# OminiX-ai/OminiX-MLX

Measured on AMD Instinct MI355X. Metric: decode_tokens_per_sec, higher is better.
Workload: dtype bf16

## Files before the change

### ominix-mlx_amd/csrc/attn_step.hip

```cpp
#include <algorithm>

#include "attn.hpp"
#include "act16.hpp"
#include "gemv_parts.hpp"
#include "granule.hpp"
#include "launch_timing.hpp"

namespace omx {

namespace {

constexpr int kBlock = 512;
constexpr int kWaves = 8;

template <int N>
__device__ __forceinline__ float swap_halves(float v) {
    if (N == 16) return dpp_f<0x128>(v);
    return dpp_f<0x1B>(dpp_f<kDppHalfMirror>(v));
}

template <bool F16 = false>
__device__ __forceinline__ void unpack8(const u32x4 r, float (&x)[8]) {
#pragma unroll
    for (int e = 0; e < 4; ++e) {
        x[2 * e] = Act16<F16>::lo(r[e]);
        x[2 * e + 1] = Act16<F16>::hi(r[e]);
    }
}

template <int D, int NB, bool F16 = false>
__device__ __forceinline__ void gather_head(const AttnStepArgs& a, const uint64_t* base, int n_active, unsigned tag, int lane,
                                            int dim, bf16_t* out, uint64_t* xg_head) {
    constexpr int STRIDE = D + 2;
    unsigned long long ml0 = 0, ml1 = 0, og[NB][16];
    bool ok_ml = false, ok_b[NB];
#pragma unroll
    for (int b = 0; b < NB; ++b) ok_b[b] = b * 16 >= n_active;
    const int sl = min(lane, n_active - 1);
    for (unsigned spins = 0;; ++spins) {
        if (!ok_ml) {
            ml0 = ld_granule(base + (size_t)sl * STRIDE + D);
            ml1 = ld_granule(base + (size_t)sl * STRIDE + D + 1);
        }
#pragma unroll
        for (int b = 0; b < NB; ++b) {
            if (ok_b[b]) continue;
#pragma unroll
            for (int j = 0; j < 16; ++j) og[b][j] = ld_granule(base + (size_t)min(b * 16 + j, n_active - 1) * STRIDE + dim);
        }
        bool all = true;
        if (!ok_ml) ok_ml = __all((unsigned)(ml0 >> 32) == tag && (unsigned)(ml1 >> 32) == tag);
        all = ok_ml;
#pragma unroll
        for (int b = 0; b < NB; ++b) {
            if (!ok_b[b]) {
                bool ok = true;
#pragma unroll
                for (int j = 0; j < 16; ++j) ok &= (unsigned)(og[b][j] >> 32) == tag;
                ok_b[b] = __all(ok);
            }
            all = all && ok_b[b];
        }
        if (all) break;
        if (spins >= kGranuleSpinLimit) {
            if (lane == 0) __hip_atomic_store(a.abort_flag, 1u, __ATOMIC_RELAXED, __HIP_MEMORY_SCOPE_AGENT);
            break;
        }
        __builtin_amdgcn_s_sleep(1);
    }
    const float m = lane < n_active ? __uint_as_float((unsigned)ml0) : -INFINITY;
    const float l = lane < n_active ? __uint_as_float((unsigned)ml1) : 0.f;
    const float M = wave_max(m);
    const float f = (m == -INFINITY) ? 0.f : __expf(m - M);
    const float L = wave_sum(f * l);
    float acc = 0.f;
#pragma unroll
    for (int b = 0; b < NB; ++b) {
        if (b * 16 >= n_active) break;
#pragma unroll
        for (int j = 0; j < 16; ++j)
            acc = fmaf(readlane_f(f, b * 16 + j), __uint_as_float((unsigned)og[b][j]), acc);
    }
    const bf16_t r = Act16<F16>::bits(acc / L);
    out[dim] = r;
    if (xg_head) {
        const float nb = dpp_f<kDppXor1>(bf16_to_f32(r));
        if (!(lane & 1)) st_granule_u32(xg_head + dim / 2, tag, (unsigned)r | ((unsigned)f32_to_bf16(nb) << 16));
    }
}

typedef __attribute__((ext_vector_type(2))) __bf16 bf16x2_t;
typedef __attribute__((ext_vector_type(2))) float f32x2;

typedef __attribute__((ext_vector_type(8))) __bf16 bf16x8_t;
__device__ __forceinline__ float dot8_bf16(const u32x4 a, const u32x4 b) {
    const bf16x8_t A = __builtin_bit_cast(bf16x8_t, a), B = __builtin_bit_cast(bf16x8_t, b);
    float d = 0.f;
    d = __builtin_amdgcn_fdot2_f32_bf16(__builtin_shufflevector(A, A, 0, 1), __builtin_shufflevector(B, B, 0, 1), d, false);
    d = __builtin_amdgcn_fdot2_f32_bf16(__builtin_shufflevector(A, A, 2, 3), __builtin_shufflevector(B, B, 2, 3), d, false);
    d = __builtin_amdgcn_fdot2_f32_bf16(__builtin_shufflevector(A, A, 4, 5), __builtin_shufflevector(B, B, 4, 5), d, false);
    d = __builtin_amdgcn_fdot2_f32_bf16(__builtin_shufflevector(A, A, 6, 7), __builtin_shufflevector(B, B, 6, 7), d, false);
    return d;
}

constexpr int kKU = 3;

template <bool F16>
__device__ __forceinline__ float dot8_16(const u32x4 a, const u32x4 b) {
    if constexpr (!F16) return dot8_bf16(a, b);
    float d = 0.f;
#pragma unroll
    for (int e = 0; e < 4; ++e) d = Act16<true>::dot2(a[e], b[e], d);
    return d;
}

constexpr int kORows = 4;

constexpr int kGuBlockPairs = 48, kGuHidden = 4096, kGuNV = kGuHidden / 512;
enum { kGuTicket = 0, kGuReduced = 1, kGuWords = 4 };

__device__ __forceinline__ int gateup_claim(int* sm_gu, int lane) {
    int t = 0;
    if (lane == 0) t = __hip_atomic_fetch_add(sm_gu + kGuTicket, 1, __ATOMIC_RELAXED, __HIP_MEMORY_SCOPE_WORKGROUP);
    return __builtin_amdgcn_readfirstlane(t);
}

__device__ __forceinline__ void gateup_issue(const AttnStepArgs& a, u32x4 (*w)[kGuNV], int pair, int lane) {
    const u32x4* g = reinterpret_cast<const u32x4*>(a.gu_gate + (size_t)pair * kGuHidden);
    const u32x4* u = reinterpret_cast<const u32x4*>(a.gu_up + (size_t)pair * kGuHidden);
#pragma unroll
    for (int j = 0; j < kGuNV; ++j) {
        w[0][j] = ld_nt(g + j * 64 + lane);
        w[1][j] = ld_nt(u + j * 64 + lane);
    }
    __builtin_amdgcn_sched_barrier(0);
}

template <int NVW>
__device__ __forceinline__ void oproj_await_vector(const AttnStepArgs& a, u32x4* sm_x, unsigned tag, int lane, int wave) {
    asm volatile("s_waitcnt vmcnt(0)" ::: "memory");
    if (wave == 0) {
        constexpr int SEGS = NVW * 8;
        const uint64_t* probe = a.xg + (size_t)min(lane, SEGS - 1) * 32 + 31;
        for (unsigned spins = 0; spins < kGranuleSpinLimit; ++spins) {
            const unsigned long long g = ld_granule(probe);
            if (__all((unsigned)(g >> 32) == tag)) break;
            __builtin_amdgcn_s_sleep(4);
        }
    }
    __syncthreads();
    constexpr int GP = (NVW + 1) / 2;
    static_assert((NVW * 256) % GP == 0, "a thread takes all of its granules or none");
    bool done = (int)threadIdx.x * GP >= NVW * 256;
    unsigned* sx = reinterpret_cast<unsigned*>(sm_x);
    for (unsigned spins = 0;; ++spins) {
        if (!done) {
            unsigned long long g[GP];
#pragma unroll
            for (int i = 0; i < GP; ++i) g[i] = ld_granule(a.xg + (size_t)threadIdx.x * GP + i);
            bool ok = true;
#pragma unroll
            for (int i = 0; i < GP; ++i) ok &= (unsigned)(g[i] >> 32) == tag;
            if (ok) {
#pragma unroll
                for (int i = 0; i < GP; ++i) sx[threadIdx.x * GP + i] = (unsigned)g[i];
                done = true;
            }
        }
        if (__syncthreads_and(done)) break;
        if (spins >= kGranuleSpinLimit) {
            if (threadIdx.x == 0) __hip_atomic_store(a.abort_flag, 1u, __ATOMIC_RELAXED, __HIP_MEMORY_SCOPE_AGENT);
            break;
        }
        __builtin_amdgcn_s_sleep(2);
    }
}

template <bool DN = false>
__device__ __forceinline__ void gateup_reduce(const AttnStepArgs& a, const u32x4 (*w)[kGuNV], const u32x4* xs, int pair, int lane,
                                              uint16_t* park = nullptr) {
    typedef Act16<false> A;
    float acc[2];
    rows_dot<false, 2, kGuNV>(w, xs, lane, acc);
    if constexpr (DN) {
        if (lane == 0) {
            const uint16_t v = epi_bits<EPI_SWIGLU, A>(acc[0], acc[1], (bf16_t)0, 0);
            a.gu_out[pair] = v;
            *park = v;
        }
    } else
    if (lane == 0) a.gu_out[pair] = epi_bits<EPI_SWIGLU, A>(acc[0], acc[1], (bf16_t)0, 0);
}

constexpr int kDnInter = 12288, kDnBlockRows = 16, kDnNV = kDnInter / 512 / 4, kDnUnits = kDnBlockRows / 2 * 4, kDnQRows = 3;
constexpr int kDnPartOff = kDnInter * 2, kDnParkOff = kDnPartOff + kDnBlockRows * 4 * 4, kDnLdsBytes = kDnParkOff + kGuBlockPairs * 2;
enum { kDnTicket = 4, kDnReduced = 5, kDnStored = 6, kDnWords = 8 };

__device__ __forceinline__ int down_claim(int* sm_gu, int lane) {
    int t = 0;
    if (lane == 0) t = __hip_atomic_fetch_add(sm_gu + kDnTicket, 1, __ATOMIC_RELAXED, __HIP_MEMORY_SCOPE_WORKGROUP);
    return __builtin_amdgcn_readfirstlane(t);
}

__device__ __forceinline__ void down_issue(const AttnStepArgs& a, u32x4 (*w)[kDnNV], int row_begin, int u, int lane) {
    const u32x4* p = reinterpret_cast<const u32x4*>(a.dn_w) + (size_t)(row_begin + 2 * (u >> 2)) * (kDnInter / 8) + (u & 3) * (kDnNV * 64) + lane;
#pragma unroll
    for (int r = 0; r < 2; ++r) {
#pragma unroll
        for (int j = 0; j < kDnNV; ++j) w[r][j] = ld_nt(p + (size_t)r * (kDnInter / 8) + j * 64);
    }
    __builtin_amdgcn_sched_barrier(0);
}

__device__ __forceinline__ void down_reduce(const u32x4 (*w)[kDnNV], const u32x4* xa, float* part, int u, int lane) {
    float acc[2];
    rows_dot<false, 2, kDnNV>(w, xa + (u & 3) * (kDnNV * 64), lane, acc);
    if (lane == 0) {
#pragma unroll
        for (int r = 0; r < 2; ++r) part[(2 * (u >> 2) + r) * 4 + (u & 3)] = acc[r];
    }
}

template <bool TRACE>
__device__ __forceinline__ void down_qkv_phase(const AttnStepArgs& a, unsigned char* sm_dn, u32x4* xs, float* red, int* sm_gu, unsigned res2,
                                               unsigned tag, int lane, int wave, unsigned long long* tr) {
    typedef Act16<false> A;
    u32x4* xa = reinterpret_cast<u32x4*>(sm_dn);
    float* part = reinterpret_cast<float*>(sm_dn + kDnPartOff);
    const int blk = (int)blockIdx.y * (int)gridDim.x + (int)blockIdx.x;
    const int row_begin = blk * kDnBlockRows;
    const int q_row0 = (blk * kWaves + __builtin_amdgcn_readfirstlane(wave)) * kDnQRows;
    constexpr int PV = kGuNV * 64 / 256;
    u32x4 nwv[PV];
#pragma unroll
    for (int i = 0; i < PV; ++i) nwv[i] = *(reinterpret_cast<const u32x4*>(a.nq_norm_w) + (threadIdx.x & 255) + i * 256);
    bf16_t ob[kDnQRows];
#pragma unroll
    for (int r = 0; r < kDnQRows; ++r) ob[r] = *(a.nq_bias ? a.nq_bias + min(q_row0 + r, a.nq.rows - 1) : a.nq_norm_w);
    u32x4 dA[2][kDnNV], dB[2][kDnNV];
    int tA = 0, tB = 0;
    u32x4 qw[kDnQRows][kGuNV];
    auto issue_qkv = [&](const int r0, const int r1) {
#pragma unroll
        for (int r = r0; r < r1; ++r) {
            const u32x4* p = reinterpret_cast<const u32x4*>(a.nq.row_ptr(min(q_row0 + r, a.nq.rows - 1), kGuHidden));
#pragma unroll
            for (int j = 0; j < kGuNV; ++j) qw[r][j] = ld_nt(p + j * 64 + lane);
        }
        __builtin_amdgcn_sched_barrier(0);
    };
    const bool sweeper = (wave & (kWaves / 2 - 1)) == 0;
    lds_barrier();
    if (wave == 0 && lane < kGuBlockPairs / 2)
        st_granule_u32(a.ag + (size_t)blk * (kGuBlockPairs / 2) + lane, tag, reinterpret_cast<const unsigned*>(sm_dn + kDnParkOff)[lane]);
    lds_barrier();
    if (sweeper) {
        constexpr int HALF = kDnInter / 2 / 2, GPL = HALF / 64;
        const int half = __builtin_amdgcn_readfirstlane(wave) / (kWaves / 2);
        const uint64_t* gr = a.ag + (size_t)half * HALF;
        for (unsigned spins = 0; spins < kGranuleSpinLimit; ++spins) {
            const unsigned long long g = ld_granule(gr + (size_t)lane * GPL + (GPL - 1));
            if (__all((unsigned)(g >> 32) == tag)) break;
            __builtin_amdgcn_s_sleep(4);
        }
        unsigned long long g[GPL];
#pragma unroll
        for (int i = 0; i < GPL; ++i) g[i] = ld_granule(gr + (size_t)i * 64 + lane);
        __builtin_amdgcn_sched_barrier(0);
        lds_barrier();
        tA = down_claim(sm_gu, lane);
        down_issue(a, dA, row_begin, tA, lane);
        unsigned bad = 0;
#pragma unroll
        for (int i = 0; i < GPL; ++i) bad |= (unsigned)(g[i] >> 32) ^ tag;
        asm volatile("; activation vector: tags read behind the first down unit" : "+v"(bad));
        if (!__all(bad == 0)) {
            for (unsigned spins = 0;; ++spins) {
#pragma unroll
                for (int i = 0; i < GPL; ++i) g[i] = ld_granule(gr + (size_t)i * 64 + lane);
                bool ok = true;
#pragma unroll
                for (int i = 0; i < GPL; ++i) ok &= (unsigned)(g[i] >> 32) == tag;
                if (__all(ok)) break;
                if (spins >= kGranuleSpinLimit) {
                    if (lane == 0) __hip_atomic_store(a.abort_flag, 1u, __ATOMIC_RELAXED, __HIP_MEMORY_SCOPE_AGENT);
                    break;
                }
                __builtin_amdgcn_s_sleep(4);
            }
        }
        unsigned* sx = reinterpret_cast<unsigned*>(xa) + half * HALF;
#pragma unroll
        for (int i = 0; i < GPL; ++i) sx[i * 64 + lane] = (unsigned)g[i];
        if (TRACE && threadIdx.x == 0) tr[11] = wall_clock64();
        tB = down_claim(sm_gu, lane);
        down_issue(a, dB, row_begin, tB, lane);
        issue_qkv(0, kDnQRows - 1);
    } else {
        tA = down_claim(sm_gu, lane);
        down_issue(a, dA, row_begin, tA, lane);
        tB = down_claim(sm_gu, lane);
        down_issue(a, dB, row_begin, tB, lane);
        issue_qkv(0, 1);
        lds_barrier();
        issue_qkv(1, kDnQRows - 1);
    }
    lds_barrier();
    down_reduce(dA, xa, part, tA, lane);
    if (TRACE && threadIdx.x == 0) tr[12] = wall_clock64();
    int n_reduced = 1;
    int nA = down_claim(sm_gu, lane), nB;
    for (;;) {
        if (nA >= kDnUnits) {
            down_reduce(dB, xa, part, tB, lane);
            ++n_reduced;
            break;
        }
        tA = nA;
        down_issue(a, dA, row_begin, tA, lane);
        nB = down_claim(sm_gu, lane);
        down_reduce(dB, xa, part, tB, lane);
        if (nB >= kDnUnits) {
            down_reduce(dA, xa, part, tA, lane);
            n_reduced += 2;
            break;
        }
        tB = nB;
        down_issue(a, dB, row_begin, tB, lane);
        nA = down_claim(sm_gu, lane);
        down_reduce(dA, xa, part, tA, lane);
        n_reduced += 2;
    }
    if (TRACE && lane == 0) __hip_atomic_fetch_add(sm_gu + kDnReduced, n_reduced, __ATOMIC_RELAXED, __HIP_MEMORY_SCOPE_WORKGROUP);
    issue_qkv(kDnQRows - 1, kDnQRows);
    lds_barrier();
    if (wave == 0) {
        if (lane < kDnBlockRows / 2) {
            const uint32_t o2 = residual_pair<A, 4>(part + 2 * lane * 4, res2);
            reinterpret_cast<uint32_t*>(a.dn_out)[row_begin / 2 + lane] = o2;
            st_granule_u32(a.rg + row_begin / 2 + lane, tag, o2);
        }
        sweep_granules<kGuHidden / 2, 1>(a.rg, reinterpret_cast<unsigned*>(xs), 0, tag, lane, a.abort_flag);
        if (TRACE && lane == 0) tr[13] = wall_clock64();
    }
    lds_barrier();
    rmsnorm_in_lds<A, PV>(xs, red, nwv, kGuHidden, a.eps, threadIdx.x < 256);
    float acc[kDnQRows];
    rows_dot<false, kDnQRows, kGuNV>(qw, xs, lane, acc);
    if (lane == 0) {
        int stored = 0;
#pragma unroll
        for (int r = 0; r < kDnQRows; ++r)
            if (q_row0 + r < a.nq.rows) {
                a.nq_out[q_row0 + r] = A::bits(a.nq_bias ? acc[r] + A::val(ob[r]) : acc[r]);
                ++stored;
            }
        if (TRACE) __hip_atomic_fetch_add(sm_gu + kDnStored, stored, __ATOMIC_RELAXED, __HIP_MEMORY_SCOPE_WORKGROUP);
    }
    if constexpr (TRACE) {
        lds_barrier();
        if (threadIdx.x == 0) {
            tr[14] = wall_clock64();
            tr[15] = (unsigned long long)sm_gu[kDnReduced] | (unsigned long long)sm_gu[kDnStored] << 32;
        }
    }
}

template <bool TRACE, bool DN = false>
__device__ __forceinline__ void gateup_phase(const AttnStepArgs& a, u32x4* xs, float* red, int* sm_gu, const uint16_t* sm_pub, unsigned tag,
                                             int lane, int wave, int pub_row0, int pub_rows, unsigned long long* tr,
                                             unsigned char* sm_dn = nullptr) {
    typedef Act16<false> A;
    const int pair0 = ((int)blockIdx.y * (int)gridDim.x + (int)blockIdx.x) * kGuBlockPairs;
    uint16_t* park = DN ? reinterpret_cast<uint16_t*>(sm_dn + kDnParkOff) : nullptr;
    constexpr int PV = kGuNV * 64 / 256;
    u32x4 nwv[PV];
#pragma unroll
    for (int i = 0; i < PV; ++i) nwv[i] = *(reinterpret_cast<const u32x4*>(a.gu_norm_w) + (threadIdx.x & 255) + i * 256);
    u32x4 wA[2][kGuNV], wB[2][kGuNV];
    int tA = 0, tB;
    if (wave != 0) {
        tA = gateup_claim(sm_gu, lane);
        gateup_issue(a, wA, pair0 + tA, lane);
    }
    lds_barrier();
    if (wave == 0) {
        if (lane < pub_rows / 2) st_granule_u32(a.hg + pub_row0 / 2 + lane, tag, reinterpret_cast<const unsigned*>(sm_pub)[lane]);
        constexpr int GPL = kGuHidden / 2 / 64;
        for (unsigned spins = 0; spins < kGranuleSpinLimit; ++spins) {
            const unsigned long long g = ld_granule(a.hg + (size_t)lane * GPL + (GPL - 1));
            if (__all((unsigned)(g >> 32) == tag)) break;
            __builtin_amdgcn_s_sleep(4);
        }
        unsigned long long g[GPL];
#pragma unroll
        for (int i = 0; i < GPL; ++i) g[i] = ld_granule(a.hg + (size_t)i * 64 + lane);
        __builtin_amdgcn_sched_barrier(0);
        lds_barrier();
        tA = gateup_claim(sm_gu, lane);
        gateup_issue(a, wA, pair0 + tA, lane);
        unsigned bad = 0;
#pragma unroll
        for (int i = 0; i < GPL; ++i) bad |= (unsigned)(g[i] >> 32) ^ tag;
        asm volatile("; hidden row: tags read behind the first (gate, up) pair" : "+v"(bad));
        if (!__all(bad == 0)) {
            for (unsigned spins = 0;; ++spins) {
#pragma unroll
                for (int i = 0; i < GPL; ++i) g[i] = ld_granule(a.hg + (size_t)i * 64 + lane);
                bool ok = true;
#pragma unroll
                for (int i = 0; i < GPL; ++i) ok &= (unsigned)(g[i] >> 32) == tag;
                if (__all(ok)) break;
                if (spins >= kGranuleSpinLimit) {
                    if (lane == 0) __hip_atomic_store(a.abort_flag, 1u, __ATOMIC_RELAXED, __HIP_MEMORY_SCOPE_AGENT);
                    break;
                }
                __builtin_amdgcn_s_sleep(4);
            }
        }
        unsigned* sx = reinterpret_cast<unsigned*>(xs);
#pragma unroll
        for (int i = 0; i < GPL; ++i) sx[i * 64 + lane] = (unsigned)g[i];
        if (TRACE && lane == 0 && pub_rows > 0) tr[4] = wall_clock64();
        tB = gateup_claim(sm_gu, lane);
    } else {
        lds_barrier();
        tB = gateup_claim(sm_gu, lane);
        gateup_issue(a, wB, pair0 + tB, lane);
    }
    lds_barrier();
    unsigned res2 = 0;
    if constexpr (DN) res2 = reinterpret_cast<const unsigned*>(xs)[(pair0 / kGuBlockPairs) * (kDnBlockRows / 2) + (lane & (kDnBlockRows / 2 - 1))];
    rmsnorm_in_lds<A, PV>(xs, red, nwv, kGuHidden, a.eps, threadIdx.x < 256);
    if (wave == 0) {
        gateup_issue(a, wB, pair0 + tB, lane);
        gateup_reduce<DN>(a, wA, xs, pair0 + tA, lane, park + tA);
        if (TRACE && threadIdx.x == 0) tr[7] = wall_clock64();
        asm volatile("; first pair reduced: wave 0, its second pair just asked for" ::: "memory");
    } else {
        gateup_reduce<DN>(a, wA, xs, pair0 + tA, lane, park + tA);
        asm volatile("; first pair reduced: the second pair came in through the hop" ::: "memory");
    }
    int n_reduced = 1;
    int nA = gateup_claim(sm_gu, lane), nB;
    for (;;) {
        if (nA >= kGuBlockPairs) {
            gateup_reduce<DN>(a, wB, xs, pair0 + tB, lane, park + tB);
            ++n_reduced;
            break;
        }
        tA = nA;
        gateup_issue(a, wA, pair0 + tA, lane);
        nB = gateup_claim(sm_gu, lane);
        gateup_reduce<DN>(a, wB, xs, pair0 + tB, lane, park + tB);
        if (nB >= kGuBlockPairs) {
            gateup_reduce<DN>(a, wA, xs, pair0 + tA, lane, park + tA);
            n_reduced += 2;
            break;
        }
        tB = nB;
        gateup_issue(a, wB, pair0 + tB, lane);
        nA = gateup_claim(sm_gu, lane);
        gateup_reduce<DN>(a, wA, xs, pair0 + tA, lane, park + tA);
        n_reduced += 2;
    }
    if constexpr (TRACE) {
        if (lane == 0) {
            __hip_atomic_fetch_add(sm_gu + kGuReduced, n_reduced, __ATOMIC_RELAXED, __HIP_MEMORY_SCOPE_WORKGROUP);
            if (wave == 0) tr[8] = wall_clock64();
            if (wave == kWaves - 1) tr[9] = wall_clock64();
        }
        lds_barrier();
        if (threadIdx.x == 0) tr[10] = (unsigned long long)sm_gu[kGuReduced];
    }
    if constexpr (DN) down_qkv_phase<TRACE>(a, sm_dn, xs, red, sm_gu, res2, tag, lane, wave, tr);
}

template <int NVW, int R, bool GU = false>
__device__ __forceinline__ void oproj_phase(const AttnStepArgs& a, u32x4* sm_x, unsigned tag, int lane, int wave, int o_row0,
                                            unsigned long long* tr, uint16_t* sm_pub = nullptr, int pub_row0 = 0) {
    u32x4 ow[R][NVW];
#pragma unroll
    for (int r = 0; r < R; ++r) {
        const int row = min(o_row0 + r, a.o_rows - 1);
        const u32x4* p = reinterpret_cast<const u32x4*>(a.o_w + (size_t)row * (NVW * 512));
#pragma unroll
        for (int j = 0; j < NVW; ++j) ow[r][j] = __builtin_nontemporal_load(p + j * 64 + lane);
    }
    bf16_t o_res[R];
#pragma unroll
    for (int r = 0; r < R; ++r) o_res[r] = a.o_resid[min(o_row0 + r, a.o_rows - 1)];
    __builtin_amdgcn_sched_barrier(0);
    oproj_await_vector<NVW>(a, sm_x, tag, lane, wave);
    if (tr && threadIdx.x == 0) tr[5] = wall_clock64();
    float acc[R];
    rows_dot<false, R, NVW>(ow, sm_x, lane, acc);
    if (lane == 0) {
#pragma unroll
        for (int r = 0; r < R; ++r)
            if (o_row0 + r < a.o_rows) {
                if (a.o_out_f32) a.o_out_f32[o_row0 + r] = acc[r];
                else {
                    const bf16_t hb = f32_to_bf16(bf16_to_f32(o_res[r]) + round_bf16(acc[r]));
                    a.o_out[o_row0 + r] = hb;
                    if (GU) sm_pub[o_row0 + r - pub_row0] = hb;
                }
            }
    }
    if (tr && threadIdx.x == 0) tr[6] = wall_clock64();
}


template <int NVW, int R>
__device__ __forceinline__ void oproj_phase_q4(const AttnStepArgs& a, u32x4* sm_x, float* sm_xsum, unsigned tag, int lane, int wave,
                                               int o_row0, unsigned long long* tr) {
    static_assert(NVW % 4 == 0, "K must be a multiple of 2048");
    constexpr int ST = NVW / 4;
    u32x4 ow[R][ST];
    uint32_t sbv[R][ST];
    const int words_per_row = NVW * 64, groups_per_row = NVW * 512 / a.o_group;
#pragma unroll
    for (int r = 0; r < R; ++r) {
        const int row = min(o_row0 + r, a.o_rows - 1);
        const uint32_t* p = a.o_wq + (size_t)row * words_per_row;
        const uint32_t* psb = a.o_sb + (size_t)row * groups_per_row;
#pragma unroll
        for (int st = 0; st < ST; ++st) {
            const int chunk = st * 64 + lane;
            ow[r][st] = __builtin_nontemporal_load(reinterpret_cast<const u32x4*>(p + (size_t)chunk * 4));
            sbv[r][st] = psb[chunk * 32 / a.o_group];
        }
    }
    bf16_t o_res[R];
#pragma unroll
    for (int r = 0; r < R; ++r) o_res[r] = a.o_resid[min(o_row0 + r, a.o_rows - 1)];
    __builtin_amdgcn_sched_barrier(0);
    oproj_await_vector<NVW>(a, sm_x, tag, lane, wave);
    if ((int)threadIdx.x < NVW * 64) {
        const u32x4 o = sm_x[threadIdx.x];
        u32x4 t;
        t[0] = __builtin_amdgcn_perm(o[1], o[0], 0x05040100u); t[1] = __builtin_amdgcn_perm(o[3], o[2], 0x05040100u);
        t[2] = __builtin_amdgcn_perm(o[1], o[0], 0x07060302u); t[3] = __builtin_amdgcn_perm(o[3], o[2], 0x07060302u);
        sm_x[threadIdx.x] = t;
        float sv = 0.f;
#pragma unroll
        for (int q = 0; q < 4; ++q) sv += bf16lo(o[q]) + bf16hi(o[q]);
        sv += dpp_f<kDppXor1>(sv);
        sv += dpp_f<kDppXor2>(sv);
        if ((threadIdx.x & 3) == 0) sm_xsum[threadIdx.x >> 2] = sv;
    }
    __syncthreads();
    if (tr && threadIdx.x == 0) tr[5] = wall_clock64();
    float acc[R];
#pragma unroll
    for (int r = 0; r < R; ++r) acc[r] = 0.f;
#pragma unroll
    for (int st = 0; st < ST; ++st) {
        const int chunk = st * 64 + lane;
        uint32_t xp[16];
#pragma unroll
        for (int j = 0; j < 4; ++j) {
            const u32x4 xv = sm_x[chunk * 4 + j];
#pragma unroll
            for (int q = 0; q < 4; ++q) xp[j * 4 + q] = xv[q];
        }
        const float xsm = sm_xsum[chunk];
#pragma unroll
        for (int r = 0; r < R; ++r) {
            float d = 0.f;
            const float scl = bf16lo(sbv[r][st]);
            float bia = bf16hi(sbv[r][st]);
#pragma unroll
            for (int wi = 0; wi < 4; ++wi) {
                const uint32_t wdw = ow[r][st][wi];
                const uint32_t lo = wdw & 0x0F0F0F0Fu, hi = (wdw >> 4) & 0x0F0F0F0Fu;
                const uint32_t c43 = 0x43434343u;
                const uint32_t q0 = __builtin_amdgcn_perm(c43, lo, 0x04010400u), q1 = __builtin_amdgcn_perm(c43, lo, 0x04030402u);
                const uint32_t q2 = __builtin_amdgcn_perm(c43, hi, 0x04010400u), q3 = __builtin_amdgcn_perm(c43, hi, 0x04030402u);
                d = __builtin_amdgcn_fdot2_f32_bf16(__builtin_bit_cast(bf16x2_t, xp[wi * 4 + 0]), __builtin_bit_cast(bf16x2_t, q0), d, false);
                d = __builtin_amdgcn_fdot2_f32_bf16(__builtin_bit_cast(bf16x2_t, xp[wi * 4 + 1]), __builtin_bit_cast(bf16x2_t, q1), d, false);
                d = __builtin_amdgcn_fdot2_f32_bf16(__builtin_bit_cast(bf16x2_t, xp[wi * 4 + 2]), __builtin_bit_cast(bf16x2_t, q2), d, false);
                d = __builtin_amdgcn_fdot2_f32_bf16(__builtin_bit_cast(bf16x2_t, xp[wi * 4 + 3]), __builtin_bit_cast(bf16x2_t, q3), d, false);
            }
            bia = fmaf(-128.0f, scl, bia);
            acc[r] = fmaf(scl, d, acc[r]);
            acc[r] = fmaf(bia, xsm, acc[r]);
        }
    }
#pragma unroll
    for (int r = 0; r < R; ++r) acc[r] = wave_sum(acc[r]);
    if (lane == 0) {
#pragma unroll
        for (int r = 0; r < R; ++r)
            if (o_row0 + r < a.o_rows) a.o_out[o_row0 + r] = f32_to_bf16(bf16_to_f32(o_res[r]) + round_bf16(acc[r]));
    }
    if (tr && threadIdx.x == 0) tr[6] = wall_clock64();
}


template <int D, int GT, bool TRACE, int NVW, bool F16 = false, bool GU = false, bool DN = false>
__global__ __launch_bounds__(kBlock, 1) void attn_step_kernel(const AttnStepArgs a) {
    static_assert(!DN || GU, "down + the next q/k/v follow gate/up only");
    static_assert(!F16 || NVW == 0, "the O projection rides in the launch for bfloat16 models only");
    static_assert(!GU || (NVW == kGuNV && D == 128), "gate/up follows the bf16 O projection of hidden 4096 only");
    typedef Act16<F16> A16;
    constexpr int LPR = D / 8;
    constexpr int TPW = 64 / LPR;
    constexpr bool QO = NVW >= 100;
    constexpr int NV = QO ? NVW - 100 : NVW;
    constexpr bool OPROJ = NV > 0;
    extern __shared__ __attribute__((aligned(16))) unsigned char smem[];
    float* sm_o = reinterpret_cast<float*>(smem);
    float* sm_m = sm_o + kWaves * TPW * GT * D;
    float* sm_l = sm_m + kWaves * GT;
    u32x4* sm_q = reinterpret_cast<u32x4*>(sm_l + kWaves * GT);
    u32x4* sm_x = sm_q + (GT + 1) * LPR;
    float* sm_xsum = reinterpret_cast<float*>(sm_x + NV * 64);
    int* sm_gu = reinterpret_cast<int*>(sm_x + NV * 64);

    const int lane = threadIdx.x & 63;
    const int wave = threadIdx.x >> 6;
    const int c = lane % LPR;
    const int sg = lane / LPR;
    const int kvh = blockIdx.x, split = blockIdx.y;
    const int G = a.H / a.Hkv;
    unsigned long long* tr = TRACE ? a.trace + ((size_t)split * a.Hkv + kvh) * kAttnTraceWords : nullptr;
    if (TRACE && threadIdx.x == 0) tr[0] = wall_clock64();
    if constexpr (GU) {
        if (threadIdx.x < (DN ? kDnWords : kGuWords)) sm_gu[threadIdx.x] = 0;
    }

    bf16_t* Kb = a.k + (size_t)kvh * a.kv_head_stride;
    bf16_t* Vb = a.v + (size_t)kvh * a.kv_head_stride;
    const int t_begin = split * a.chunk;
    const int n_units = a.chunk / TPW;

    const bf16_t* kraw = a.qkv + (size_t)a.H * D + (size_t)kvh * D;
    const bool does_q = wave < GT, does_k = wave == GT % kWaves;
    const bf16_t* my_raw = does_q ? a.qkv + (size_t)(kvh * G + min(wave, G - 1)) * D : kraw;
    const u32x4 raw0 = *reinterpret_cast<const u32x4*>(my_raw + c * 8);
    const u32x4 raw1 = *reinterpret_cast<const u32x4*>(kraw + c * 8);
    const u32x4 vnew = *reinterpret_cast<const u32x4*>(kraw + (size_t)a.Hkv * D + c * 8);
    const int i0 = (c % (LPR / 2)) * 8;
    const f32x4* cp = reinterpret_cast<const f32x4*>(a.rope_cur + i0);
    const f32x4* sp = reinterpret_cast<const f32x4*>(a.rope_cur + D / 2 + i0);
    const f32x4 c0 = cp[0], c1 = cp[1], s0 = sp[0], s1 = sp[1];
    u32x4 wq_raw = {0, 0, 0, 0}, wk_raw = {0, 0, 0, 0};
    if (a.q_norm_w) {
        wq_raw = *reinterpret_cast<const u32x4*>(a.q_norm_w + c * 8);
        wk_raw = *reinterpret_cast<const u32x4*>(a.k_norm_w + c * 8);
    }
    u32x4 kr[kKU], vr[kKU];
    auto issue_kv = [&](int u0) {
#pragma unroll
        for (int u = 0; u < kKU; ++u) {
            const int tc = min(t_begin + (u0 + u * kWaves) * TPW + sg, a.cap - 1);
            kr[u] = *reinterpret_cast<const u32x4*>(Kb + (size_t)tc * D + c * 8);
            vr[u] = *reinterpret_cast<const u32x4*>(Vb + (size_t)tc * D + c * 8);
        }
    };
    issue_kv(wave);
    const int pos = *a.pos_ptr;
    const unsigned tag = *a.seq_ptr * a.tag_mul + a.tag_add;

    {
        float cs[8], sn[8];
#pragma unroll
        for (int e = 0; e < 4; ++e) {
            cs[e] = c0[e]; cs[4 + e] = c1[e];
            sn[e] = s0[e]; sn[4 + e] = s1[e];
        }
        const bool first_half = c < LPR / 2;
        auto norm_rope = [&](const u32x4 raw, const u32x4 w_raw) -> u32x4 {
            float x[8], w[8];
            unpack8<F16>(raw, x);
            unpack8<F16>(w_raw, w);
            float ss = 0.f;
#pragma unroll
            for (int e = 0; e < 8; ++e) ss = fmaf(x[e], x[e], ss);
            ss = group_sum<LPR>(ss);
            const float rstd = a.q_norm_w ? 1.0f / sqrtf(ss / (float)D + a.eps) : 1.0f;
            float y[8];
#pragma unroll
            for (int e = 0; e < 8; ++e) {
                const float xn = a.q_norm_w ? A16::rnd(x[e] * rstd * w[e]) : x[e];
                const float other = swap_halves<LPR>(xn);
                y[e] = first_half ? xn * cs[e] - other * sn[e] : other * sn[e] + xn * cs[e];
            }
            u32x4 out;
#pragma unroll
            for (int e = 0; e < 4; ++e) out[e] = A16::pack(y[2 * e], y[2 * e + 1]);
            return out;
        };
        if (does_q && sg == 0) sm_q[wave * LPR + c] = norm_rope(raw0, wq_raw);
        if (does_k && sg == 0) sm_q[GT * LPR + c] = norm_rope(does_q ? raw1 : raw0, wk_raw);
    }
    asm volatile("s_waitcnt lgkmcnt(0)\n\ts_barrier" ::: "memory");
    u32x4 q[GT];
#pragma unroll
    for (int g = 0; g < GT; ++g) q[g] = sm_q[g * LPR + c];
    const u32x4 knew = sm_q[GT * LPR + c];

    const int Tk = pos + 1;
    const int n_active = (Tk + a.chunk - 1) / a.chunk;
    const int t_end = min(Tk, t_begin + a.chunk);
    const bool active = split < n_active;
    if (TRACE && threadIdx.x == 0) tr[1] = wall_clock64();

    float m[GT], l[GT];
    f32x2 o[GT][4];
#pragma unroll
    for (int g = 0; g < GT; ++g) {
        m[g] = -INFINITY;
        l[g] = 0.f;
#pragma unroll
        for (int e = 0; e < 4; ++e) o[g][e] = f32x2{0.f, 0.f};
    }
    auto round = [&](const int u0) {
        float s[kKU][GT];
        f32x2 vf[kKU][4];
#pragma unroll
        for (int u = 0; u < kKU; ++u) {
            const int unit = u0 + u * kWaves;
            const int tok = t_begin + unit * TPW + sg;
            const bool live = unit < n_units && tok < t_end;
            u32x4 kp = kr[u], vp = vr[u];
            if (tok == pos && unit < n_units) {
                kp = knew;
                vp = vnew;
                *reinterpret_cast<u32x4*>(Kb + (size_t)pos * D + c * 8) = kp;
                *reinterpret_cast<u32x4*>(Vb + (size_t)pos * D + c * 8) = vp;
            }
#pragma unroll
            for (int e = 0; e < 4; ++e)
                vf[u][e] = live ? f32x2{A16::lo(vp[e]), A16::hi(vp[e])} : f32x2{0.f, 0.f};
#pragma unroll
            for (int g = 0; g < GT; ++g) {
                const float d = group_sum<LPR>(dot8_16<F16>(q[g], kp)) * a.scale;
                s[u][g] = live ? d : -INFINITY;
            }
        }
        if (u0 + kWaves * kKU < n_units && t_begin + (u0 + kWaves * kKU) * TPW < t_end) issue_kv(u0 + kWaves * kKU);
#pragma unroll
        for (int g = 0; g < GT; ++g) {
            float mx = s[0][g];
#pragma unroll
            for (int u = 1; u < kKU; ++u) mx = fmaxf(mx, s[u][g]);
            float wmx = readlane_f(mx, 0);
#pragma unroll
            for (int r = 1; r < TPW; ++r) wmx = fmaxf(wmx, readlane_f(mx, r * LPR));
            const float mn = fmaxf(m[g], wmx);
            const float alpha = (mn == -INFINITY) ? 1.f : __expf(m[g] - mn);
            m[g] = mn;
            l[g] *= alpha;
            const f32x2 al = {alpha, alpha};
#pragma unroll
            for (int e = 0; e < 4; ++e) o[g][e] *= al;
#pragma unroll
            for (int u = 0; u < kKU; ++u) {
                const float p = (mn == -INFINITY) ? 0.f : __expf(s[u][g] - mn);
                l[g] += p;
                const f32x2 pp = {p, p};
#pragma unroll
                for (int e = 0; e < 4; ++e) o[g][e] = __builtin_elementwise_fma(pp, vf[u][e], o[g][e]);
            }
        }
    };
    if (wave < n_units && t_begin + wave * TPW < t_end) round(wave);
    for (int u0 = wave + kWaves * kKU; u0 < n_units && t_begin + u0 * TPW < t_end; u0 += kWaves * kKU) round(u0);
    if (TRACE && threadIdx.x == 0) tr[2] = wall_clock64();

    if (active) {
#pragma unroll
        for (int g = 0; g < GT; ++g) {
            float* dst = sm_o + (((size_t)(wave * TPW + sg) * GT + g) * D + c * 8);
            *reinterpret_cast<f32x4*>(dst) = f32x4{o[g][0][0], o[g][0][1], o[g][1][0], o[g][1][1]};
            *reinterpret_cast<f32x4*>(dst + 4) = f32x4{o[g][2][0], o[g][2][1], o[g][3][0], o[g][3][1]};
            float lw = readlane_f(l[g], 0);
#pragma unroll
            for (int r = 1; r < TPW; ++r) lw += readlane_f(l[g], r * LPR);
            if (lane == 0) {
                sm_m[wave * GT + g] = m[g];
                sm_l[wave * GT + g] = lw;
            }
        }
        __syncthreads();
        if (TRACE && !GU && threadIdx.x == 0) tr[7] = wall_clock64();
        for (int idx = threadIdx.x; idx < G * D; idx += kBlock) {
            const int g = idx / D, d = idx % D;
            float M = sm_m[g];
#pragma unroll
            for (int w = 1; w < kWaves; ++w) M = fmaxf(M, sm_m[w * GT + g]);
            float L = 0.f, O = 0.f;
#pragma unroll
            for (int w = 0; w < kWaves; ++w) {
                const float mw = sm_m[w * GT + g];
                const float f = (mw == -INFINITY) ? 0.f : __expf(mw - M);
                float ow = 0.f;
#pragma unroll
                for (int r = 0; r < TPW; ++r) ow += sm_o[((size_t)(w * TPW + r) * GT + g) * D + d];
                L = fmaf(f, sm_l[w * GT + g], L);
                O = fmaf(f, ow, O);
            }
            uint64_t* gr = a.ws + ((size_t)(kvh * G + g) * a.nsplit + split) * (D + 2);
            st_granule(gr + d, tag, O);
            if (d == 0) {
                st_granule(gr + D, tag, M);
                st_granule(gr + D + 1, tag, L);
            }
        }
    }
    if (TRACE && threadIdx.x == 0) tr[3] = wall_clock64();

    if (OPROJ && split >= G) {
        const int g = ((split - G) * (int)gridDim.x + kvh) * kWaves + wave;
        const bool hi = g < a.o_nhi;
        const int rows = hi ? a.o_rpw : a.o_rpw - 1;
        const int o_row0 = hi ? g * a.o_rpw : a.o_nhi * a.o_rpw + (g - a.o_nhi) * (a.o_rpw - 1);
        unsigned long long* otr = TRACE ? tr : nullptr;
        if constexpr (GU) {
            auto row0_of = [&](int w) { return w < a.o_nhi ? w * a.o_rpw : a.o_nhi * a.o_rpw + (w - a.o_nhi) * (a.o_rpw - 1); };
            const int pub_row0 = row0_of(g - wave), pub_rows = row0_of(g - wave + kWaves) - pub_row0;
            uint16_t* sm_pub = reinterpret_cast<uint16_t*>(sm_l);
            if (rows == 2) oproj_phase<NV, 2, true>(a, sm_x, tag, lane, wave, o_row0, otr, sm_pub, pub_row0);
            else oproj_phase<NV, 3, true>(a, sm_x, tag, lane, wave, o_row0, otr, sm_pub, pub_row0);
            gateup_phase<TRACE, DN>(a, sm_x, sm_m, sm_gu, sm_pub, tag, lane, wave, pub_row0, pub_rows, otr, smem);
            return;
        } else
        if constexpr (QO) {
            if (rows <= 1) oproj_phase_q4<NV, 1>(a, sm_x, sm_xsum, tag, lane, wave, o_row0, otr);
            else if (rows == 2) oproj_phase_q4<NV, 2>(a, sm_x, sm_xsum, tag, lane, wave, o_row0, otr);
            else if (rows == 3) oproj_phase_q4<NV, 3>(a, sm_x, sm_xsum, tag, lane, wave, o_row0, otr);
            else oproj_phase_q4<NV, 4>(a, sm_x, sm_xsum, tag, lane, wave, o_row0, otr);
        } else {
            if (rows <= 1) oproj_phase<(NV > 0 ? NV : 1), 1>(a, sm_x, tag, lane, wave, o_row0, otr);
            else if (rows == 2) oproj_phase<(NV > 0 ? NV : 1), 2>(a, sm_x, tag, lane, wave, o_row0, otr);
            else if (rows == 3) oproj_phase<(NV > 0 ? NV : 1), 3>(a, sm_x, tag, lane, wave, o_row0, otr);
            else oproj_phase<(NV > 0 ? NV : 1), 4>(a, sm_x, tag, lane, wave, o_row0, otr);
        }
        return;
    }

    if (split < G && wave < D / 64) {
        const int head = kvh * G + split;
        const uint64_t* base = a.ws + (size_t)head * a.nsplit * (D + 2);
        bf16_t* out = a.out + (size_t)head * D;
        const int dim = wave * 64 + lane;
        const int nb = (a.nsplit + 15) / 16;
        uint64_t* xg_head = OPROJ ? a.xg + (size_t)head * (D / 2) : nullptr;
        if (nb <= 1) gather_head<D, 1, F16>(a, base, n_active, tag, lane, dim, out, xg_head);
        else if (nb == 2) gather_head<D, 2, F16>(a, base, n_active, tag, lane, dim, out, xg_head);
        else gather_head<D, 3, F16>(a, base, n_active, tag, lane, dim, out, xg_head);
        if (TRACE && threadIdx.x == 0) tr[4] = wall_clock64();
    }
    if constexpr (GU) {
        lds_barrier();
        gateup_phase<TRACE, DN>(a, sm_x, sm_m, sm_gu, nullptr, tag, lane, wave, 0, 0, TRACE ? tr : nullptr, smem);
    }
}

}

int attn_step_block_tokens(int D) { return 64 / (D / 8); }

constexpr int kMaxSplits = 48;
void attn_step_plan(int tk_max, int Hkv, int G, int D, int* chunk, int* nsplit) {
    const int unit = attn_step_block_tokens(D);
    int target = std::max(1, std::min(kMaxSplits, 256 / std::max(Hkv, 1)));
    if (const char* v = getenv("OMX_ATTN_STEP_SPLITS")) target = std::max(1, std::min(kMaxSplits, atoi(v)));
    int ch = unit * ((tk_max + unit * target - 1) / (unit * target));
    if (ch < unit) ch = unit;
    int ns = (tk_max + ch - 1) / ch;
    if (ns < G) ns = G;
    *chunk = ch;
    *nsplit = ns;
}

size_t attn_step_ws_granules(int H, int D) { return (size_t)H * kMaxSplits * (D + 2); }

static int oproj_rows_per_wave(int H, int Hkv, int nsplit, int o_rows) {
    const int waves = (Hkv * nsplit - H) * kWaves;
    return waves > 0 ? (o_rows + waves - 1) / waves : 1 << 20;
}
bool attn_step_oproj_ok(int H, int Hkv, int D, int nsplit, int o_rows) {
    const int K = H * D, nvw = K / 512;
    return K % 512 == 0 && (nvw == 1 || nvw == 2 || nvw == 4 || nvw == 7 || nvw == 8) && oproj_rows_per_wave(H, Hkv, nsplit, o_rows) <= kORows;
}

bool attn_step_oproj_q4_ok(int H, int Hkv, int D, int nsplit, int o_rows, int group) {
    const int K = H * D;
    return (K == 2048 || K == 4096) && (group == 32 || group == 64 || group == 128) && attn_step_oproj_ok(H, Hkv, D, nsplit, o_rows);
}

bool attn_step_gateup_ok(int H, int Hkv, int D, int nsplit, int o_rows, int gu_rows) {
    const int blocks = Hkv * nsplit, waves = (blocks - H) * kWaves;
    if (D != 128 || H * D != kGuHidden || o_rows != kGuHidden || H / std::max(Hkv, 1) != 4 || blocks != 256) return false;
    if (gu_rows != blocks * kGuBlockPairs || !attn_step_oproj_ok(H, Hkv, D, nsplit, o_rows)) return false;
    return oproj_rows_per_wave(H, Hkv, nsplit, o_rows) == 3 && (o_rows - waves * 2) % kWaves == 0;
}

bool attn_step_down_ok(int o_rows, int gu_rows, int nq_rows) {
    const int waves = 256 * kWaves;
    return o_rows == 256 * kDnBlockRows && gu_rows == kDnInter && nq_rows > (kDnQRows - 1) * waves && nq_rows <= kDnQRows * waves;
}

template <int D, int GT, bool TRACE, int NVW, bool F16 = false, bool GU = false, bool DN = false>
static int launch_instance(dim3 grid, size_t shmem, hipStream_t s, const AttnStepArgs& a) {
    if (shmem > 48 * 1024)
        OMX_HIP_CHECK(hipFuncSetAttribute((const void*)attn_step_kernel<D, GT, TRACE, NVW, F16, GU, DN>, hipFuncAttributeMaxDynamicSharedMemorySize, (int)shmem));
    OMX_LAUNCH_TIMED((attn_step_kernel<D, GT, TRACE, NVW, F16, GU, DN>), grid, dim3(kBlock), shmem, s, a);
    OMX_LAUNCH_CHECK();
    return 0;
}

int launch_attn_step(const AttnStepArgs& a_in, int D, hipStream_t s) {
    AttnStepArgs a = a_in;
    const int G = a.H / a.Hkv;
    OMX_REQUIRE(a.H % a.Hkv == 0 && G >= 1 && G <= 8, "decode attention: %d query heads over %d KV heads unsupported (group of at most 8)", a.H, a.Hkv);
    OMX_REQUIRE(a.nsplit >= G && a.nsplit <= kMaxSplits && a.chunk > 0 && a.chunk % attn_step_block_tokens(D) == 0 && a.Hkv * a.nsplit <= 256,
                "decode attention: bad split plan (chunk %d, %d splits, group %d, %d kv heads)", a.chunk, a.nsplit, G, a.Hkv);
    OMX_REQUIRE(a.ws && a.rope_cur && a.pos_ptr && a.seq_ptr && a.abort_flag && a.tag_mul > a.tag_add - 1u && a.tag_add >= 1u,
                "decode attention: missing step state");
    int nvw = 0;
    const bool qo = a.o_wq != nullptr;
    if (qo)
        OMX_REQUIRE(!a.o_w && a.o_sb && a.o_out && !a.o_out_f32 && attn_step_oproj_q4_ok(a.H, a.Hkv, D, a.nsplit, a.o_rows, a.o_group),
                    "decode attention + packed O projection: shape does not qualify (H*D = %d, group %d)", a.H * D, a.o_group);
    if (a.o_w || qo) {
        OMX_REQUIRE(a.o_resid && (a.o_out || a.o_out_f32) && a.xg && attn_step_oproj_ok(a.H, a.Hkv, D, a.nsplit, a.o_rows),
                    "decode attention + O projection: shape does not qualify (H*D = %d, %d rows, %d blocks)", a.H * D, a.o_rows, a.Hkv * a.nsplit);
        nvw = a.H * D / 512;
        a.o_rpw = oproj_rows_per_wave(a.H, a.Hkv, a.nsplit, a.o_rows);
        const int waves = (a.Hkv * a.nsplit - a.H) * kWaves;
        a.o_nhi = a.o_rpw > 1 ? a.o_rows - waves * (a.o_rpw - 1) : waves;
    }
    if (a.gu_gate)
        OMX_REQUIRE(a.o_w && a.o_out && !a.o_out_f32 && !a.f16 && a.gu_up && a.gu_norm_w && a.gu_out && a.hg &&
                        attn_step_gateup_ok(a.H, a.Hkv, D, a.nsplit, a.o_rows, a.gu_rows),
                    "decode attention + gate/up: shape does not qualify (%d blocks, %d O rows, %d pairs)", a.Hkv * a.nsplit, a.o_rows, a.gu_rows);
    if (a.dn_w)
        OMX_REQUIRE(a.gu_gate && a.dn_out && a.ag && a.rg && a.nq.w0 && a.nq.w1 && a.nq.w2 && a.nq_norm_w && a.nq_out &&
                        a.nq.n0 > 0 && a.nq.n1 > 0 && a.nq.rows > a.nq.n0 + a.nq.n1 && attn_step_down_ok(a.o_rows, a.gu_rows, a.nq.rows),
                    "decode attention + down + q/k/v: shape does not qualify (%d rows, %d pairs, %d q/k/v rows)", a.o_rows, a.gu_rows, a.nq.rows);
    const dim3 grid(a.Hkv, a.nsplit);
    const int gt = G <= 1 ? 1 : G <= 2 ? 2 : G <= 4 ? 4 : 8;
#define OMX_ATTN_STEP_CASE(DD, GG)                                                                                       \
    if (D == DD && gt == GG) {                                                                                           \
        const size_t shmem = ((size_t)kWaves * (64 / (DD / 8)) * GG * DD + 2 * kWaves * GG) * sizeof(float) +            \
                             (size_t)(GG + 1) * (DD / 8) * 16 + (size_t)nvw * 64 * 16 + (qo ? (size_t)nvw * 64 : 0) +    \
                             (a.dn_w ? kDnWords * sizeof(int) : a.gu_gate ? kGuWords * sizeof(int) : 0);                 \
        if (a.gu_gate) {                            \
            if constexpr (DD == 128 && GG == 4) {                                                                        \
                static_assert(kDnLdsBytes <= kWaves * 4 * 4 * 128 * 4, "the down phase lives in the split-merge area");  \
                if (a.dn_w && a.trace) return launch_instance<128, 4, true, kGuNV, false, true, true>(grid, shmem, s, a); \
                if (a.dn_w) return launch_instance<128, 4, false, kGuNV, false, true, true>(grid, shmem, s, a);          \
                if (a.trace) return launch_instance<128, 4, true, kGuNV, false, true>(grid, shmem, s, a);                \
                return launch_instance<128, 4, false, kGuNV, false, true>(grid, shmem, s, a);                            \
            }                                                                                                            \
            return set_error("decode attention + gate/up: no instantiation for head_dim %d, group %d", DD, GG);         \
        }                                                                                                                \
        if (a.trace && !qo) {                           \
            if (nvw == 0) return launch_instance<DD, GG, true, 0>(grid, shmem, s, a);                                    \
            if (nvw == 8) return launch_instance<DD, GG, true, 8>(grid, shmem, s, a);                                    \
            return set_error("decode attention: no traced instantiation for H*D = %d", a.H * DD);                       \
        }                                                                                                                \
        if (qo) {                                                                                                        \
            if (nvw == 4) return launch_instance<DD, GG, false, 104>(grid, shmem, s, a);                                 \
            return launch_instance<DD, GG, false, 108>(grid, shmem, s, a);                                               \
        }                                                                                                                \
        if (a.f16) {    \
            if constexpr (DD == 128) {                                                                                   \
                if (nvw == 0) return launch_instance<DD, GG, false, 0, true>(grid, shmem, s, a);                         \
            }                                                                                                            \
            return set_error("decode attention: float16 models take head_dim 128 without the O projection in the launch"); \
        }                                                                                                                \
        if (nvw == 0) return launch_instance<DD, GG, false, 0>(grid, shmem, s, a);                                       \
        if (nvw == 1) return launch_instance<DD, GG, false, 1>(grid, shmem, s, a);                                       \
        if (nvw == 2) return launch_instance<DD, GG, false, 2>(grid, shmem, s, a);                                       \
        if (nvw == 4) return launch_instance<DD, GG, false, 4>(grid, shmem, s, a);                                       \
        if (nvw == 7) return launch_instance<DD, GG, false, 7>(grid, shmem, s, a);                                       \
        return launch_instance<DD, GG, false, 8>(grid, shmem, s, a);                                                     \
    }
    OMX_ATTN_STEP_CASE(128, 1) OMX_ATTN_STEP_CASE(128, 2) OMX_ATTN_STEP_CASE(128, 4) OMX_ATTN_STEP_CASE(128, 8)
    OMX_ATTN_STEP_CASE(64, 1) OMX_ATTN_STEP_CASE(64, 2) OMX_ATTN_STEP_CASE(64, 4) OMX_ATTN_STEP_CASE(64, 8)
#undef OMX_ATTN_STEP_CASE
    return set_error("decode attention: head_dim %d unsupported (64 or 128)", D);
}

}
```

Before: 357.8.

## Defer q/k/v weight loads until after down-reduce and overlap with residual sweep

Stops issuing the q/k/v projection weight loads early, where they competed with the down-projection loads and held registers. All q/k/v rows are now issued together once the down reduction finishes. Wave 0 first issues its residual granule loads and then the q/k/v loads, so the weight fetch overlaps the residual tag wait, with a spin-retry fallback. This shortens the register live range and the memory contention during the down phase, but gives up overlap of the weight loads with down-projection work.

```diff
diff --git a/ominix-mlx_amd/csrc/attn_step.hip b/ominix-mlx_amd/csrc/attn_step.hip
--- a/ominix-mlx_amd/csrc/attn_step.hip
+++ b/ominix-mlx_amd/csrc/attn_step.hip
@@ -240,9 +240,9 @@
     u32x4 dA[2][kDnNV], dB[2][kDnNV];
     int tA = 0, tB = 0;
     u32x4 qw[kDnQRows][kGuNV];
-    auto issue_qkv = [&](const int r0, const int r1) {
-#pragma unroll
-        for (int r = r0; r < r1; ++r) {
+    auto issue_qkv = [&]() {
+#pragma unroll
+        for (int r = 0; r < kDnQRows; ++r) {
             const u32x4* p = reinterpret_cast<const u32x4*>(a.nq.row_ptr(min(q_row0 + r, a.nq.rows - 1), kGuHidden));
 #pragma unroll
             for (int j = 0; j < kGuNV; ++j) qw[r][j] = ld_nt(p + j * 64 + lane);
@@ -295,15 +295,12 @@
         if (TRACE && threadIdx.x == 0) tr[11] = wall_clock64();
         tB = down_claim(sm_gu, lane);
         down_issue(a, dB, row_begin, tB, lane);
-        issue_qkv(0, kDnQRows - 1);
     } else {
         tA = down_claim(sm_gu, lane);
         down_issue(a, dA, row_begin, tA, lane);
         tB = down_claim(sm_gu, lane);
         down_issue(a, dB, row_begin, tB, lane);
-        issue_qkv(0, 1);
         lds_barrier();
-        issue_qkv(1, kDnQRows - 1);
     }
     lds_barrier();
     down_reduce(dA, xa, part, tA, lane);
@@ -332,16 +329,46 @@
         n_reduced += 2;
     }
     if (TRACE && lane == 0) __hip_atomic_fetch_add(sm_gu + kDnReduced, n_reduced, __ATOMIC_RELAXED, __HIP_MEMORY_SCOPE_WORKGROUP);
-    issue_qkv(kDnQRows - 1, kDnQRows);
     lds_barrier();
+    if (wave == 0 && lane < kDnBlockRows / 2) {
+        const uint32_t o2 = residual_pair<A, 4>(part + 2 * lane * 4, res2);
+        reinterpret_cast<uint32_t*>(a.dn_out)[row_begin / 2 + lane] = o2;
+        st_granule_u32(a.rg + row_begin / 2 + lane, tag, o2);
+    }
     if (wave == 0) {
-        if (lane < kDnBlockRows / 2) {
-            const uint32_t o2 = residual_pair<A, 4>(part + 2 * lane * 4, res2);
-            reinterpret_cast<uint32_t*>(a.dn_out)[row_begin / 2 + lane] = o2;
-            st_granule_u32(a.rg + row_begin / 2 + lane, tag, o2);
-        }
-        sweep_granules<kGuHidden / 2, 1>(a.rg, reinterpret_cast<unsigned*>(xs), 0, tag, lane, a.abort_flag);
+        constexpr int GPL = kGuHidden / 2 / 64;
+        unsigned long long g[GPL];
+#pragma unroll
+        for (int i = 0; i < GPL; ++i) g[i] = ld_granule(a.rg + (size_t)i * 64 + lane);
+        __builtin_amdgcn_sched_barrier(0);
+        lds_barrier();
+        issue_qkv();
+        unsigned bad = 0;
+#pragma unroll
+        for (int i = 0; i < GPL; ++i) bad |= (unsigned)(g[i] >> 32) ^ tag;
+        asm volatile("; residual row: tags read behind wave 0's q/k/v rows" : "+v"(bad));
+        if (!__all(bad == 0)) {
+            for (unsigned spins = 0;; ++spins) {
+#pragma unroll
+                for (int i = 0; i < GPL; ++i) g[i] = ld_granule(a.rg + (size_t)i * 64 + lane);
+                bool ok = true;
+#pragma unroll
+                for (int i = 0; i < GPL; ++i) ok &= (unsigned)(g[i] >> 32) == tag;
+                if (__all(ok)) break;
+                if (spins >= kGranuleSpinLimit) {
+                    if (lane == 0) __hip_atomic_store(a.abort_flag, 1u, __ATOMIC_RELAXED, __HIP_MEMORY_SCOPE_AGENT);
+                    break;
+                }
+                __builtin_amdgcn_s_sleep(4);
+            }
+        }
+        unsigned* sx = reinterpret_cast<unsigned*>(xs);
+#pragma unroll
+        for (int i = 0; i < GPL; ++i) sx[i * 64 + lane] = (unsigned)g[i];
         if (TRACE && lane == 0) tr[13] = wall_clock64();
+    } else {
+        lds_barrier();
+        issue_qkv();
     }
     lds_barrier();
     rmsnorm_in_lds<A, PV>(xs, red, nwv, kGuHidden, a.eps, threadIdx.x < 256);
```

New measurement: 367.3 (median of 6 runs). 1.03x the previous value.
